# A-SHOJAEI/adverse-weather-semantic-segmentation-robustness-benchmark

Hardware: AMD Instinct MI355X
Metric: images/sec (1024x2048, 5 weather conds, ensemble eval) (higher is better)
Workload: dtype f32 (results float32; attention, gemm_1x1, winograd_3x3, segformer_head on 3xf16 split operands: 22-bit operands, f32 accumulate)

## Files before the change

adverse_weather_semantic_segmentation_robustness_benchmark_amd/_native.py:

```python
from __future__ import annotations

import ctypes as C
from pathlib import Path

import numpy as np
import torch

_PKG = Path(__file__).resolve().parent
LIB_PATH = _PKG / "libawseg_hip.so"

U8, I64 = 0, 1
COMBINE_WEIGHTED, COMBINE_MAXCONF, COMBINE_MEAN = 0, 1, 2
LOSS_CE, LOSS_FOCAL = 0, 1
ACT_NONE, ACT_RELU, ACT_GELU = 0, 1, 2
MAX_CLASSES = 32

c_i, c_i64, c_u64, c_f, c_d, c_p = C.c_int, C.c_int64, C.c_uint64, C.c_float, C.c_double, C.c_void_p

FOG_JOB = np.dtype([("image", "<i4"), ("_pad", "<i4"), ("beta", "<f8"), ("atmos", "<f8"), ("seed", "<u8")], align=True)
NIGHT_JOB = np.dtype([("image", "<i4"), ("_pad", "<i4"), ("brightness", "<f8"), ("intensity", "<f8"), ("seed", "<u8")], align=True)
PRIM_JOB = np.dtype([("image", "<i4"), ("prim_offset", "<i4"), ("prim_count", "<i4"), ("blur_ksize", "<i4"), ("intensity", "<f8")], align=True)
WEATHER_JOB = np.dtype([("kind", "<i4"), ("image", "<i4"), ("a", "<f8"), ("b", "<f8"), ("seed", "<u8"), ("prim_offset", "<i4"), ("prim_count", "<i4")], align=True)
WEATHER_CLEAN, WEATHER_FOG, WEATHER_RAIN, WEATHER_SNOW, WEATHER_NIGHT = 0, 1, 2, 3, 4
assert FOG_JOB.itemsize == 32 and NIGHT_JOB.itemsize == 32 and PRIM_JOB.itemsize == 24 and WEATHER_JOB.itemsize == 40
# ... 12 lines not shown
    "awseg_normalize": (c_i, [c_p, c_i64, c_i, c_i, c_p, c_i, c_p, c_p, c_p, c_p]),
    "awseg_synthetic_depth": (c_i, [c_i, c_i, c_p, c_i, c_p, c_p, c_p, c_p]),
    "awseg_conv3x3_winograd_nhwc": (c_i, [c_p, c_i, c_i, c_i, c_i, c_i, c_i, c_p, c_p, c_p, c_i, c_p, c_p, c_p, c_p]),
    "awseg_gemm_bias_act": (c_i, [c_p, c_p, c_p, c_p, c_i, c_p, c_i64, c_i, c_i, c_p, C.c_size_t, c_p]),
    "awseg_gemm_tune": (c_i, [c_p, c_p, c_p, c_i, c_i, c_p, c_i64, c_i, c_i, c_p, C.c_size_t, c_p]),
    "awseg_gemm_split_weights": (c_i, [c_p, c_i, c_i, c_p, c_p]),
    "awseg_gemm_split_weight_halfs": (c_i64, [c_i, c_i]),
    "awseg_gemm_split_bias_act": (c_i, [c_p, c_p, c_p, c_p, c_i, c_p, c_i64, c_i, c_i, c_p]),
    "awseg_gemm_bf16_weights": (c_i, [c_p, c_i, c_i, c_p, c_p]),
    "awseg_gemm_bf16_weight_halfs": (c_i64, [c_i, c_i]),
    "awseg_gemm_bf16_bias_act": (c_i, [c_p, c_p, c_p, c_p, c_i, c_p, c_i64, c_i, c_i, c_p]),
    "awseg_conv3x3_winograd_bf16_nhwc": (c_i, [c_p, c_i, c_i, c_i, c_i, c_i, c_i, c_p, c_p, c_p, c_i, c_p, c_p, c_p, c_p]),
    "awseg_attention_d32_bf16": (c_i, [c_p, c_p, c_p, c_p, c_i, c_i, c_i, c_i, c_f, c_p]),
    "awseg_attention_d32_split_workspace": (c_i64, [c_i, c_i, c_i]),
    "awseg_attention_d32_split_ws": (c_i, [c_p, c_p, c_p, c_i, c_p, c_i, c_i, c_i, c_i, c_f, c_p, c_p]),
    "awseg_attention_d32_packed_kv": (c_i, [c_p, c_p, c_p, c_i, c_i, c_i, c_i, c_f, c_i, c_p]),
    "awseg_dwconv3x3_upcat_nhwc": (c_i, [c_p, c_i, c_i, c_i, c_p, c_i, c_i64, c_i, c_i, c_p, c_p, c_p]),
    "awseg_winograd_split_weight_halfs": (c_i64, [c_i, c_i]),
    "awseg_conv3x3_winograd_split_nhwc": (c_i, [c_p, c_i, c_i, c_i, c_i, c_i, c_i, c_p, c_p, c_p, c_i, c_p, c_p, c_p, c_p]),
    "awseg_upconv_forms_floats": (c_i64, [c_i, c_i, c_i]),
    "awseg_upconv_forms": (c_i, [c_p, c_i, c_i, c_i, c_i, c_p, c_p, c_p]),
    "awseg_depth_head_fused": (c_i, [c_p, c_i, c_i, c_i, c_i, c_p, c_i, c_p, c_p, c_p, c_p, c_p]),
    "awseg_im2col_nhwc": (c_i, [c_p, c_i64, c_i, c_i, c_i, c_i, c_i, c_i, c_i, c_i, c_i, c_p, c_p]),
    "awseg_attention_d32": (c_i, [c_p, c_p, c_p, c_p, c_i, c_i, c_i, c_i, c_f, c_p]),
    "awseg_attention_d32_split": (c_i, [c_p, c_p, c_p, c_p, c_i, c_i, c_i, c_i, c_f, c_p]),
    "awseg_depth_upsample_combine": (c_i, [c_p, c_p, c_i, c_i, c_i, c_i, c_i, c_p, c_p, c_p, c_p]),
    "awseg_lut3_apply": (c_i, [c_p, c_i, c_i, c_i, c_p, c_i, c_p, c_p, c_p]),
    "awseg_local_contrast": (c_i, [c_p, c_i, c_i, c_i, c_p, c_p]),
    "awseg_depth_estimate_workspace": (C.c_size_t, [c_i]),
    "awseg_depth_estimate": (c_i, [c_p, c_i, c_i, c_i, c_p, c_p, c_p, c_p, c_p]),
# ... 173 lines not shown
```

adverse_weather_semantic_segmentation_robustness_benchmark_amd/csrc/attn.hip:

```cpp
#include "awseg_common.h"

namespace {

typedef float f32x16 __attribute__((ext_vector_type(16)));

constexpr int AT = 256;
#ifndef AWSEG_ATTN_SPLIT_WAVES
#define AWSEG_ATTN_SPLIT_WAVES 2
#endif
constexpr int D = 32;
constexpr int TK = 32;
constexpr int LDK = 36;

__device__ __forceinline__ constexpr int acc_row(int r, int hk) { return (r & 3) + 8 * (r >> 2) + 4 * hk; }

__global__ __launch_bounds__(AT, 2)
void attention_d32_kernel(const float* __restrict__ q, const float* __restrict__ k, const float* __restrict__ v,
                          float* __restrict__ out, int nq, int nkv, int heads, float scale_log2e, int kvp)
{
    __shared__ float sK[2][TK * LDK];
    __shared__ float sV[2][D * LDK];
    const int tid = threadIdx.x, lane = tid & 63, wave = tid >> 6;
    const int hk = lane >> 5, li = lane & 31;
    const int h = blockIdx.y, b = blockIdx.z;
// ... 362 lines not shown
    if (!attn_split_pass<false>(q, k, v, out, nq, nkv, heads, scale_log2e, kvp, sK, sV, sMax, one)) return;
    const int eq = guard_exponent(sMax[0]), ek = guard_exponent(sMax[1]), ev = guard_exponent(sMax[2]);
    auto p2 = [](int e) { return __builtin_bit_cast(float, (unsigned)(127 + e) << 23); };
    const attn_scales sc = {p2(-eq), p2(-ek), p2(-ev), p2(eq), p2(ek), p2(ev)};
    attn_split_pass<true>(q, k, v, out, nq, nkv, heads, scale_log2e, kvp, sK, sV, sMax, sc);
}

constexpr int IMG_TILE_HALFS = (TK + D) * SROW;

__device__ __forceinline__ uint32_t at_lds_addr(const void* p) { return (uint32_t)(uintptr_t)(__attribute__((address_space(3))) const void*)p; }
__device__ __forceinline__ void at_dma16(__amdgpu_buffer_rsrc_t rsrc, uint32_t voff, uint32_t soff, uint32_t lds_base)
{
    asm volatile("s_mov_b32 m0, %3\n\ts_nop 0\n\tbuffer_load_dwordx4 %0, %1, %2 offen lds" : : "v"(voff), "s"(rsrc), "s"(soff), "s"(lds_base) : "m0", "memory");
}

__global__ __launch_bounds__(AT)
void attn_kv_image_kernel(const float* __restrict__ k, const float* __restrict__ v, int kvp, int nkv, int heads,
                          _Float16* __restrict__ img, int* __restrict__ exps)
{
    __shared__ unsigned sM[2];
    const int tid = threadIdx.x, h = blockIdx.x, b = blockIdx.y;
    const float* kb = k + (size_t)b * nkv * kvp + h * D;
    const float* vb = v + (size_t)b * nkv * kvp + h * D;
    const int lkey = tid >> 3, lc = tid & 7;
    const size_t g_off = (size_t)lkey * kvp + 4 * lc;
    const int wk0 = lkey * SROW + 4 * lc;
    const int wv0 = TK * SROW + (4 * lc) * SROW + pv_slot(lkey);
    const int ntiles = nkv / TK;
    if (tid < 2) sM[tid] = 0u;
    __syncthreads();
    float kmax = 0.f, vmax = 0.f;
    for (int t = 0; t < ntiles; ++t) {
        kmax = amax4(kmax, *reinterpret_cast<const float4*>(kb + (size_t)t * TK * kvp + g_off));
        vmax = amax4(vmax, *reinterpret_cast<const float4*>(vb + (size_t)t * TK * kvp + g_off));
    }
    if (kmax >= kSplitLimit) atomicMax(&sM[0], __builtin_bit_cast(unsigned, kmax));
    if (vmax >= kSplitLimit) atomicMax(&sM[1], __builtin_bit_cast(unsigned, vmax));
    __syncthreads();
    const int ek = guard_exponent(sM[0]), ev = guard_exponent(sM[1]);
    auto p2 = [](int e) { return __builtin_bit_cast(float, (unsigned)(127 + e) << 23); };
    const float sk = p2(-ek), sv = p2(-ev);
    if (tid == 0) { exps[((size_t)b * heads + h) * 2] = ek; exps[((size_t)b * heads + h) * 2 + 1] = ev; }
    _Float16* base = img + ((size_t)b * heads + h) * ntiles * IMG_TILE_HALFS;
    for (int t = 0; t < ntiles; ++t) {
        float4 kk4 = *reinterpret_cast<const float4*>(kb + (size_t)t * TK * kvp + g_off);
        float4 vv4 = *reinterpret_cast<const float4*>(vb + (size_t)t * TK * kvp + g_off);
        kk4.x *= sk; kk4.y *= sk; kk4.z *= sk; kk4.w *= sk;
        vv4.x *= sv; vv4.y *= sv; vv4.z *= sv; vv4.w *= sv;
        _Float16* T = base + (size_t)t * IMG_TILE_HALFS;
        u32x2 H, L; unsigned hh, ll;
        split_pair(kk4.x, kk4.y, hh, ll); H[0] = hh; L[0] = ll;
        split_pair(kk4.z, kk4.w, hh, ll); H[1] = hh; L[1] = ll;
        *reinterpret_cast<u32x2*>(&T[wk0]) = H;
        *reinterpret_cast<u32x2*>(&T[wk0 + 32]) = L;
        unsigned vh01, vl01, vh23, vl23;
        split_pair(vv4.x, vv4.y, vh01, vl01);
        split_pair(vv4.z, vv4.w, vh23, vl23);
        unsigned short* sv16 = reinterpret_cast<unsigned short*>(&T[wv0]);
        sv16[0] = (unsigned short)vh01;            sv16[32] = (unsigned short)vl01;
        sv16[SROW] = (unsigned short)(vh01 >> 16); sv16[SROW + 32] = (unsigned short)(vl01 >> 16);
        sv16[2 * SROW] = (unsigned short)vh23;     sv16[2 * SROW + 32] = (unsigned short)vl23;
        sv16[3 * SROW] = (unsigned short)(vh23 >> 16); sv16[3 * SROW + 32] = (unsigned short)(vl23 >> 16);
    }
}

template <bool SCALED, bool QGUARD>
__device__ __forceinline__ bool attn_split_pass_img(const float* __restrict__ q, const _Float16* __restrict__ img_bh, float* __restrict__ out,
                                                    int nq, int nkv, int heads, float scale_log2e, _Float16 (*sKV)[IMG_TILE_HALFS],
                                                    unsigned* sMax, const attn_scales sc)
{
    const int tid = threadIdx.x, lane = tid & 63, wave = tid >> 6;
    const int hk = lane >> 5, li = lane & 31;
    const int h = blockIdx.y, b = blockIdx.z;
    const int C = heads * D;
    const int q0 = blockIdx.x * 128 + wave * 32;
    float qmax = 0.f;
    h8 qh[2], ql[2];
    {
        const int qi = q0 + li;
        const float* qp = q + ((size_t)b * nq + (qi < nq ? qi : nq - 1)) * C + h * D;
        const float qs = SCALED ? scale_log2e * sc.sq : scale_log2e;
#pragma unroll
        for (int s = 0; s < 2; ++s) {
            const float4 a4 = *reinterpret_cast<const float4*>(qp + 16 * s + 8 * hk);
            const float4 b4 = *reinterpret_cast<const float4*>(qp + 16 * s + 8 * hk + 4);
            const float x[8] = { a4.x * qs, a4.y * qs, a4.z * qs, a4.w * qs, b4.x * qs, b4.y * qs, b4.z * qs, b4.w * qs };
            if (QGUARD) {
#pragma unroll
                for (int i = 0; i < 8; ++i) qmax = __builtin_fmaxf(qmax, __builtin_fabsf(x[i]));
            }
            split8(x, qh[s], ql[s]);
        }
    }
// ... 4 lines not shown
    auto dma_tile = [&](int t, int buf) {
        const uint32_t so = (uint32_t)t * (uint32_t)(IMG_TILE_HALFS * 2), lb = lds0 + (uint32_t)buf * (uint32_t)(IMG_TILE_HALFS * 2);
        at_dma16(rsrc, (uint32_t)(lane * 16) + wave_u * 1024u, so, lb + wave_u * 1024u);
        at_dma16(rsrc, (uint32_t)(lane * 16) + (wave_u + 4u) * 1024u, so, lb + (wave_u + 4u) * 1024u);
        if (wave_u == 0) at_dma16(rsrc, (uint32_t)(lane * 16) + 8192u, so, lb + 8192u);
    };
    dma_tile(0, 0);
    asm volatile("s_waitcnt vmcnt(0)" ::: "memory");
    __syncthreads();

    f32x16 om, oc;
#pragma unroll
    for (int r = 0; r < 16; ++r) { om[r] = 0.f; oc[r] = 0.f; }
    float m_run = -1e30f, l_run = 0.f;
    const int a_off = li * SROW + 8 * hk;

    for (int t = 0; t < ntiles; ++t) {
        const int buf = t & 1;
        if (t + 1 < ntiles) dma_tile(t + 1, buf ^ 1);
        const h8* kr = reinterpret_cast<const h8*>(&sKV[buf][a_off]);
        const h8 kh0 = kr[0], kh1 = kr[2], kl0 = kr[4], kl1 = kr[6];
        f32x16 sm, scx;
#pragma unroll
        for (int r = 0; r < 16; ++r) { sm[r] = 0.f; scx[r] = 0.f; }
        sm = __builtin_amdgcn_mfma_f32_32x32x16_f16(kh0, qh[0], sm, 0, 0, 0);
        scx = __builtin_amdgcn_mfma_f32_32x32x16_f16(kh0, ql[0], scx, 0, 0, 0);
        sm = __builtin_amdgcn_mfma_f32_32x32x16_f16(kh1, qh[1], sm, 0, 0, 0);
        scx = __builtin_amdgcn_mfma_f32_32x32x16_f16(kh1, ql[1], scx, 0, 0, 0);
        scx = __builtin_amdgcn_mfma_f32_32x32x16_f16(kl0, qh[0], scx, 0, 0, 0);
        scx = __builtin_amdgcn_mfma_f32_32x32x16_f16(kl1, qh[1], scx, 0, 0, 0);
        const h8* vr = reinterpret_cast<const h8*>(&sKV[buf][TK * SROW + a_off]);
        const h8 vh0 = vr[0], vh1 = vr[2], vl0 = vr[4], vl1 = vr[6];
        float s[16];
#pragma unroll
        for (int r = 0; r < 16; ++r) {
            s[r] = fmaf(scx[r], kLoInv, sm[r]);
            if (SCALED) s[r] = s[r] * sc.bq * sc.bk;
        }
        float mt = fmaxf(fmaxf(s[0], s[1]), fmaxf(s[2], s[3]));
#pragma unroll
        for (int r = 4; r < 16; r += 4) mt = fmaxf(mt, fmaxf(fmaxf(s[r], s[r + 1]), fmaxf(s[r + 2], s[r + 3])));
        mt = fmaxf(mt, __shfl_xor(mt, 32, 64));
        const float m_new = fmaxf(m_run, mt);
        const float alpha = __builtin_amdgcn_exp2f(m_run - m_new);
        const float m_sh = m_new - 15.0f;
        float p[16], ls = 0.f;
// ... 11 lines not shown
        split8_unscaled(p + 8, ph1, pl1);
        om = __builtin_amdgcn_mfma_f32_32x32x16_f16(vh0, ph0, om, 0, 0, 0);
        oc = __builtin_amdgcn_mfma_f32_32x32x16_f16(vl0, ph0, oc, 0, 0, 0);
        om = __builtin_amdgcn_mfma_f32_32x32x16_f16(vh1, ph1, om, 0, 0, 0);
        oc = __builtin_amdgcn_mfma_f32_32x32x16_f16(vl1, ph1, oc, 0, 0, 0);
        om = __builtin_amdgcn_mfma_f32_32x32x16_f16(vh0, pl0, om, 0, 0, 0);
        om = __builtin_amdgcn_mfma_f32_32x32x16_f16(vh1, pl1, om, 0, 0, 0);
        asm volatile("s_waitcnt vmcnt(0)" ::: "memory");
        __syncthreads();
    }

    if (QGUARD) {
        if (qmax >= kSplitLimit) atomicMax(&sMax[0], __builtin_bit_cast(unsigned, qmax));
        __syncthreads();
        if (sMax[0] != 0u) return true;
    }
    const int qi = q0 + li;
    if (qi < nq) {
        const float inv = 1.0f / l_run;
        float* op = out + ((size_t)b * nq + qi) * C + h * D;
#pragma unroll
        for (int g = 0; g < 4; ++g) {
            float4 o4 = make_float4(fmaf(oc[4 * g], kLoInv, om[4 * g]) * inv, fmaf(oc[4 * g + 1], kLoInv, om[4 * g + 1]) * inv,
                                    fmaf(oc[4 * g + 2], kLoInv, om[4 * g + 2]) * inv, fmaf(oc[4 * g + 3], kLoInv, om[4 * g + 3]) * inv);
            if (SCALED) { o4.x *= sc.bv; o4.y *= sc.bv; o4.z *= sc.bv; o4.w *= sc.bv; }
            *reinterpret_cast<float4*>(op + 8 * g + 4 * hk) = o4;
        }
    }
    return false;
}
// ... 8 lines not shown
    if (threadIdx.x == 0) sMax[0] = 0u;
    const _Float16* img_bh = img + ((size_t)b * heads + h) * (size_t)(nkv / TK) * IMG_TILE_HALFS;
    const int ek = exps[((size_t)b * heads + h) * 2], ev = exps[((size_t)b * heads + h) * 2 + 1];
    auto p2 = [](int e) { return __builtin_bit_cast(float, (unsigned)(127 + e) << 23); };
    attn_scales sc = {1.f, p2(-ek), p2(-ev), 1.f, p2(ek), p2(ev)};
    bool redo;
    if ((ek | ev) == 0) redo = attn_split_pass_img<false, true>(q, img_bh, out, nq, nkv, heads, scale_log2e, sKV, sMax, sc);
    else redo = attn_split_pass_img<true, true>(q, img_bh, out, nq, nkv, heads, scale_log2e, sKV, sMax, sc);
    if (!redo) return;
    const int eq = guard_exponent(sMax[0]);
    sc.sq = p2(-eq); sc.bq = p2(eq);
    __syncthreads();
    attn_split_pass_img<true, false>(q, img_bh, out, nq, nkv, heads, scale_log2e, sKV, sMax, sc);
}

__global__ __launch_bounds__(AT, 2)
void attention_d32_bf16_kernel(const float* __restrict__ q, const float* __restrict__ k, const float* __restrict__ v,
                               float* __restrict__ out, int nq, int nkv, int heads, float scale_log2e, int kvp)
{
    __shared__ __attribute__((aligned(16))) _Float16 sK[2][TK * SROW];
    __shared__ __attribute__((aligned(16))) _Float16 sV[2][D * SROW];
    __shared__ unsigned sMax[3];
    const attn_scales one = {1.f, 1.f, 1.f, 1.f, 1.f, 1.f};
    attn_split_pass<false, true>(q, k, v, out, nq, nkv, heads, scale_log2e, kvp, sK, sV, sMax, one);
}

}

namespace {
template <typename K>
// ... 42 lines not shown

AWSEG_API int awseg_attention_d32_split_ws(const float* q, const float* k, const float* v, int kv_pitch, float* out, int batch, int heads,
                                           int n_queries, int n_keys, float scale, void* workspace, awseg_stream_t stream)
{
    if (batch == 0 || n_queries == 0) return 0;
    if (!q || !k || !v || !out || !workspace || batch < 0 || heads < 1 || n_queries < 0 || n_keys < TK) return AWSEG_EINVAL;
    if (n_keys % TK) return AWSEG_ERANGE;
    if (heads > 65535 || batch > 65535) return AWSEG_ERANGE;
    if (((uintptr_t)q & 15) || ((uintptr_t)k & 15) || ((uintptr_t)v & 15) || ((uintptr_t)out & 15) || ((uintptr_t)workspace & 255)) return AWSEG_EALIGN;
    if (kv_pitch == 0) kv_pitch = heads * D;
    if (kv_pitch < heads * D || (kv_pitch & 3)) return AWSEG_EINVAL;
    if ((int64_t)(n_keys / TK) * IMG_TILE_HALFS * 2 > 0x7fffffff) return AWSEG_ERANGE;
    int* exps = reinterpret_cast<int*>(workspace);
    const int64_t tab = ((int64_t)batch * heads * 2 * 4 + 255) / 256 * 256;
    _Float16* img = reinterpret_cast<_Float16*>(reinterpret_cast<char*>(workspace) + tab);
    hipLaunchKernelGGL(attn_kv_image_kernel, dim3((unsigned)heads, (unsigned)batch), dim3(AT), 0, awseg_s(stream), k, v, kv_pitch, n_keys, heads, img, exps);
    AWSEG_LAUNCH_CHECK();
    dim3 grid((unsigned)((n_queries + 127) / 128), (unsigned)heads, (unsigned)batch);
    hipLaunchKernelGGL(attention_d32_split_img_kernel, grid, dim3(AT), 0, awseg_s(stream), q, img, exps, out, n_queries, n_keys, heads,
                       scale * 1.4426950408889634f);
    AWSEG_LAUNCH_CHECK();
    return 0;
}

AWSEG_API int awseg_attention_d32_packed_kv(const float* q, const float* kv, float* out, int batch, int heads, int n_queries,
                                            int n_keys, float scale, int mode, awseg_stream_t stream)
{
    if (!kv) return AWSEG_EINVAL;
    const int c = heads * D;
    switch (mode) {
    case 0: return launch_attention(attention_d32_kernel, q, kv, kv + c, out, batch, heads, n_queries, n_keys, scale, stream, 2 * c);
    case 1: return launch_attention(attention_d32_split_kernel, q, kv, kv + c, out, batch, heads, n_queries, n_keys, scale, stream, 2 * c);
    case 2: return launch_attention(attention_d32_bf16_kernel, q, kv, kv + c, out, batch, heads, n_queries, n_keys, scale, stream, 2 * c);
    default: return AWSEG_EINVAL;
    }
// ... 2 lines not shown
```

adverse_weather_semantic_segmentation_robustness_benchmark_amd/models/fused.py:

```python
from __future__ import annotations

import contextlib
import os
from typing import List

import torch
import torch.nn as nn
import torch.nn.functional as F

from .. import _native as N
from .. import ops

CL = torch.channels_last


def _pair(v):
    return (v, v) if isinstance(v, int) else tuple(v)


def _versions(*tensors):
    return tuple((t.data_ptr(), t._version) for t in tensors if t is not None)


DERIVED = ("wsplit", "wbf16", "wsplit_small", "kvsplit", "proj_pieces", "stemrows")
# ... 339 lines not shown
    if lin.bias is not None and x.is_contiguous() and (ops.gemm_wants_bf16(m, lin.out_features, k) or
                                                       (LINEAR_SPLIT and ops.gemm_wants_split(m, lin.out_features, k))):
        y = ops.gemm_bias_act(x.view(m, k), lin.weight, lin.bias, N.ACT_NONE, w_split=split_weights(lin, lin.weight, m))
        return y.view(*x.shape[:-1], lin.out_features)
    return F.linear(x, lin.weight, lin.bias)


def _linear_residual(x2: torch.Tensor, lin: nn.Linear, tok: torch.Tensor) -> torch.Tensor:
    if lin.bias is None or not tok.is_contiguous():
        return tok + F.linear(x2, lin.weight, lin.bias).view_as(tok)
    t2 = tok.view(-1, tok.shape[-1])
    ops.gemm_bias_act(x2, lin.weight, lin.bias, N.ACT_NONE, residual=t2, out=t2, w_split=split_weights(lin, lin.weight, x2.shape[0]))
    return tok


def _kv_packed(kv: torch.Tensor, a) -> torch.Tensor:
    kp, vp = a.k_proj, a.v_proj
    wkv, bkv = cached(a, "kvpack", [kp.weight, kp.bias, vp.weight, vp.bias],
                      lambda: (torch.cat([kp.weight, vp.weight]).contiguous(), torch.cat([kp.bias, vp.bias]).contiguous()))
    c = kv.shape[-1]
    m = kv.numel() // c
    if ops.gemm_wants_bf16(m, 2 * c, c) or ops.gemm_wants_split(m, 2 * c, c):
        y = ops.gemm_bias_act(kv.view(m, c), wkv, bkv, N.ACT_NONE, w_split=split_weights(a, wkv, m))
    else:
        ws = cached(a, "kvsplit", (wkv,), lambda: ops.gemm_split_weights(wkv))
        y = ops.gemm_bias_act(kv.view(m, c), wkv, bkv, N.ACT_NONE, w_split=ws, split=True)
    return y.view(*kv.shape[:-1], 2 * c)


@torch.no_grad()
# ... 5 lines not shown
    for st in seg.stages:
        pe = st.patch_embeddings
        if _is_patch_gemm(pe.proj) and pe.proj.bias is not None:
            w2 = cached(pe.proj, "patch", [pe.proj.weight], lambda: patch_weights(pe.proj))
            y = conv_gemm_nhwc(nhwc_view(t), pe.proj, w2, pe.proj.bias, N.ACT_NONE)
        else:
            y = _stem_rows(t, pe.proj, pe.proj.weight, pe.proj.bias) if pe.proj.bias is not None else None
            if y is None:
                w = cached(pe.proj, "wcl", [pe.proj.weight], lambda: pe.proj.weight.contiguous(memory_format=CL))
                y = nhwc_view(F.conv2d(t.contiguous(memory_format=CL), w, pe.proj.bias, pe.proj.stride, pe.proj.padding))
        tok = _ln(y, pe.layer_norm)
        B, H, W, C = tok.shape
        for blk in st.blocks:
            a = blk.attention
            hcur = _ln(tok, blk.layernorm_before)
            q = _linear(hcur, a.q_proj)
            if a.sequence_reduction_ratio > 1:
                sr = a.sequence_reduction
                src = sr.sequence_reduction
                if _is_patch_gemm(src) and src.bias is not None:
                    w2 = cached(src, "patch", [src.weight], lambda: patch_weights(src))
                    kv = conv_gemm_nhwc(hcur, src, w2, src.bias, N.ACT_NONE)
                else:
                    wsr = cached(src, "wcl", [src.weight], lambda: src.weight.contiguous(memory_format=CL))
                    kv = nhwc_view(F.conv2d(hcur.permute(0, 3, 1, 2), wsr, src.bias, src.stride))
                kv = _ln(kv, sr.layer_norm)
            else:
                kv = hcur
            nh, d = a.num_attention_heads, a.head_dim
            nkv = kv.shape[1] * kv.shape[2]
            if (d == 32 and nkv % 32 == 0 and ops.KV_PACKED and kv.is_cuda and kv.dtype == torch.float32 and C % 8 == 0
                    and a.k_proj.bias is not None and a.v_proj.bias is not None and kv.is_contiguous()):
                o = ops.attention_d32_packed_kv(q.view(B, H * W, C), _kv_packed(kv, a).view(B, nkv, 2 * C), nh, a.scaling).view(B * H * W, C)
            elif d == 32 and nkv % 32 == 0:
                k, v = _linear(kv, a.k_proj), _linear(kv, a.v_proj)
                o = ops.attention_d32(q.view(B, H * W, C), k.reshape(B, nkv, C), v.reshape(B, nkv, C), nh, a.scaling).view(B * H * W, C)
            else:
                k, v = _linear(kv, a.k_proj), _linear(kv, a.v_proj)
                qq, kk, vv = (t_.view(B, -1, nh, d).transpose(1, 2) for t_ in (q.view(B, H * W, C), k.reshape(B, -1, C), v.reshape(B, -1, C)))
                if ops.PRECISION == "bf16":
                    o = F.scaled_dot_product_attention(qq.bfloat16(), kk.bfloat16(), vv.bfloat16(), scale=a.scaling).float()
                else:
                    o = F.scaled_dot_product_attention(qq, kk, vv, scale=a.scaling)
                o = o.transpose(1, 2).reshape(B * H * W, C)
            tok = _linear_residual(o, a.o_proj, tok)
            m = blk.mlp
            ln2 = blk.layernorm_after
            if (ops.MIXFFN_FUSED and tok.is_cuda and tok.dtype == torch.float32 and C in (32, 64)
                    and getattr(seg.config, "hidden_act", "gelu") == "gelu" and m.fc1.bias is not None and m.fc2.bias is not None
                    and m.dwconv.dwconv.bias is not None and ln2.weight is not None and ln2.bias is not None):
                prep = cached(m, "mixffn", [ln2.weight, ln2.bias, m.fc1.weight, m.fc2.weight],
                              lambda: (ops.mixffn_split_weights(m.fc1.weight), ops.mixffn_split_weights(m.fc2.weight))
                              if ops.mixffn_operands_ok(ln2.weight, ln2.bias, m.fc1.weight, m.fc2.weight) else None)
                fusedtok = None if prep is None else ops.mixffn_fused(
                    tok, ln2.weight, ln2.bias, ln2.eps, m.fc1.weight, m.fc1.bias, dw_taps(m.dwconv.dwconv), m.dwconv.dwconv.bias,
                    m.fc2.weight, m.fc2.bias, w1_split=prep[0], w2_split=prep[1], checked=True)
                if fusedtok is not None:
                    tok = fusedtok
                    continue
            hcur = _linear(_ln(tok, blk.layernorm_after), m.fc1)
# ... 9 lines not shown
```

adverse_weather_semantic_segmentation_robustness_benchmark_amd/ops.py:

```python
from __future__ import annotations

import math
import os

import ctypes as C
from typing import Optional, Sequence

import numpy as np
import torch

from . import _native as N

IMAGENET_MEAN = np.array([0.485, 0.456, 0.406], dtype=np.float32)
IMAGENET_STD = np.array([0.229, 0.224, 0.225], dtype=np.float32)
NIGHT_GAINS = np.array([0.8, 0.85, 1.2], dtype=np.float32)
CONDITIONS = ("clean", "fog", "rain", "snow", "night")


def gaussian_taps(sigma: float = 2.0, truncate: float = 4.0) -> np.ndarray:
    radius = int(truncate * float(sigma) + 0.5)
    x = np.arange(-radius, radius + 1)
    phi = np.exp(-0.5 / (sigma * sigma) * x ** 2)
    return phi / phi.sum()

# ... 1221 lines not shown
    if split is None and PRECISION == "bf16":
        sym = "awseg_attention_d32_bf16"
    else:
        sym = "awseg_attention_d32_split" if (ATTENTION_SPLIT if split is None else split) else "awseg_attention_d32"
    if sym == "awseg_attention_d32_split" and _wants_kv_image(nq, k.shape[1]):
        _attention_split_ws(q, k, v, 0, out, b, heads, nq, k.shape[1], scale)
        return out
    N.call(sym, N.ptr(q), N.ptr(k), N.ptr(v), N.ptr(out), b, heads, nq, k.shape[1], float(scale), N.stream())
    return out


ATTN_KV_IMAGE = os.environ.get("AWSEG_ATTN_KV_IMAGE", "1") != "0"


def _wants_kv_image(nq: int, nkv: int) -> bool:
    return ATTN_KV_IMAGE and nq >= 8 * nkv


def _attention_split_ws(q, k, v, pitch, out, b, heads, nq, nkv, scale):
    nbytes = int(N.lib().awseg_attention_d32_split_workspace(b, heads, nkv))
    ws = N.workspace.get(q.device, nbytes, tag="attn%d" % torch.cuda.current_stream(q.device).cuda_stream)
    N.call("awseg_attention_d32_split_ws", N.ptr(q), N.ptr_strided(k), N.ptr_strided(v), int(pitch), N.ptr(out), b, heads, nq, nkv, float(scale),
           N.ptr(ws), N.stream())


def attention_d32_packed_kv(q: torch.Tensor, kv: torch.Tensor, heads: int, scale: float, split: Optional[bool] = None) -> torch.Tensor:
    q, kv = q.contiguous(), kv.contiguous()
    b, nq, c = q.shape
    assert kv.shape[-1] == 2 * c
    out = torch.empty_like(q)
    mode = 2 if (split is None and PRECISION == "bf16") else (1 if (ATTENTION_SPLIT if split is None else split) else 0)
    if mode == 1 and _wants_kv_image(nq, kv.shape[1]):
        _attention_split_ws(q, kv, kv[..., c:], 2 * c, out, b, heads, nq, kv.shape[1], scale)
        return out
    N.call("awseg_attention_d32_packed_kv", N.ptr(q), N.ptr(kv), N.ptr(out), b, heads, nq, kv.shape[1], float(scale), mode, N.stream())
    return out


# ... 140 lines not shown
```

include/awseg.h:

```cpp
#ifndef AWSEG_H
#define AWSEG_H

#include <stddef.h>
#include <stdint.h>

#ifdef __cplusplus
extern "C" {
#endif

typedef void* awseg_stream_t;

#define AWSEG_EINVAL   (-1)
#define AWSEG_ERANGE   (-2)
#define AWSEG_EALIGN   (-3)

#define AWSEG_U8   0
#define AWSEG_I64  1

#define AWSEG_COMBINE_WEIGHTED  0
#define AWSEG_COMBINE_MAXCONF   1
#define AWSEG_COMBINE_MEAN      2

#define AWSEG_LOSS_CE     0
#define AWSEG_LOSS_FOCAL  1
// ... 218 lines not shown
                                        const float* bias, const float* residual, int act, float* out, int n,
                                        awseg_stream_t stream);

int64_t awseg_gemm_bf16_weight_halfs(int n, int k);
int awseg_gemm_bf16_weights(const float* w, int n, int k, uint16_t* w_bf16, awseg_stream_t stream);
int awseg_gemm_bf16_bias_act(const float* x, const uint16_t* w_bf16, const float* bias, const float* residual, int act,
                             float* out, int64_t m, int n, int k, awseg_stream_t stream);
int awseg_conv3x3_winograd_bf16_nhwc(const float* x, int batch, int height, int width, int cin, int cout, int dilation,
                                     const uint16_t* u_bf16, const float* shift, const float* residual, int act,
                                     const float* w2, const float* b2, float* out, awseg_stream_t stream);
int awseg_attention_d32_bf16(const float* q, const float* k, const float* v, float* out, int batch, int heads,
                             int n_queries, int n_keys, float scale, awseg_stream_t stream);
int64_t awseg_attention_d32_split_workspace(int batch, int heads, int n_keys);
int awseg_attention_d32_split_ws(const float* q, const float* k, const float* v, int kv_pitch, float* out, int batch, int heads,
                                 int n_queries, int n_keys, float scale, void* workspace, awseg_stream_t stream);

int awseg_attention_d32_packed_kv(const float* q, const float* kv, float* out, int batch, int heads, int n_queries,
                                  int n_keys, float scale, int mode, awseg_stream_t stream);

int awseg_upconv3x3_linear(const float* g9, int64_t batch, int cmid, int h, int w, int height, int width,
                           const float* bias, float* out, int channels_last, awseg_stream_t stream);
int awseg_upconv3x3_adjoint(const float* dz, int64_t batch, int cmid, int h, int w, int height, int width,
                            float* dg9, awseg_stream_t stream);

int awseg_im2col_nhwc(const float* x, int64_t batch, int height, int width, int channels, int kernel_h, int kernel_w,
                      int stride, int pad, int dilation, int k_padded, float* cols, awseg_stream_t stream);

int awseg_attention_d32(const float* q, const float* k, const float* v, float* out, int batch, int heads,
                        int n_queries, int n_keys, float scale, awseg_stream_t stream);

// ... 159 lines not shown
```

Baseline: 235.6.

## Fuse Q and output projections into the single-head d32 attention kernel

Adds a fused attention kernel for single-head, 32-channel stages. It computes the Q projection from the layernorm output in registers via split-f16 MFMA, runs the KV-image attention, then applies the output projection plus residual directly into the token buffer. This removes two separate GEMM launches and the round trips of q and o through global memory. The KV image builder is also spread across several tile-blocks per head and stages tiles in LDS for coalesced stores, and the KV-image threshold is lowered to nq >= 4*nkv. The cost is more register pressure and extra in-kernel block reductions for the dynamic input scaling.

```diff
diff --git a/adverse_weather_semantic_segmentation_robustness_benchmark_amd/_native.py b/adverse_weather_semantic_segmentation_robustness_benchmark_amd/_native.py
--- a/adverse_weather_semantic_segmentation_robustness_benchmark_amd/_native.py
+++ b/adverse_weather_semantic_segmentation_robustness_benchmark_amd/_native.py
@@ -50,6 +50,7 @@
     "awseg_attention_d32_bf16": (c_i, [c_p, c_p, c_p, c_p, c_i, c_i, c_i, c_i, c_f, c_p]),
     "awseg_attention_d32_split_workspace": (c_i64, [c_i, c_i, c_i]),
     "awseg_attention_d32_split_ws": (c_i, [c_p, c_p, c_p, c_i, c_p, c_i, c_i, c_i, c_i, c_f, c_p, c_p]),
+    "awseg_attention_d32_proj_ws": (c_i, [c_p, c_p, c_p, c_p, c_p, c_p, c_p, c_i, c_p, c_i, c_i, c_i, c_i, c_i, c_f, c_p, c_p]),
     "awseg_attention_d32_packed_kv": (c_i, [c_p, c_p, c_p, c_i, c_i, c_i, c_i, c_f, c_i, c_p]),
     "awseg_dwconv3x3_upcat_nhwc": (c_i, [c_p, c_i, c_i, c_i, c_p, c_i, c_i64, c_i, c_i, c_p, c_p, c_p]),
     "awseg_winograd_split_weight_halfs": (c_i64, [c_i, c_i]),
diff --git a/adverse_weather_semantic_segmentation_robustness_benchmark_amd/csrc/attn.hip b/adverse_weather_semantic_segmentation_robustness_benchmark_amd/csrc/attn.hip
--- a/adverse_weather_semantic_segmentation_robustness_benchmark_amd/csrc/attn.hip
+++ b/adverse_weather_semantic_segmentation_robustness_benchmark_amd/csrc/attn.hip
@@ -400,12 +400,15 @@
     asm volatile("s_mov_b32 m0, %3\n\ts_nop 0\n\tbuffer_load_dwordx4 %0, %1, %2 offen lds" : : "v"(voff), "s"(rsrc), "s"(soff), "s"(lds_base) : "m0", "memory");
 }
 
+constexpr int IMG_TILES_PER_BLOCK = 4;
+
 __global__ __launch_bounds__(AT)
 void attn_kv_image_kernel(const float* __restrict__ k, const float* __restrict__ v, int kvp, int nkv, int heads,
                           _Float16* __restrict__ img, int* __restrict__ exps)
 {
+    __shared__ __attribute__((aligned(16))) _Float16 sT[2][IMG_TILE_HALFS];
     __shared__ unsigned sM[2];
-    const int tid = threadIdx.x, h = blockIdx.x, b = blockIdx.y;
+    const int tid = threadIdx.x, h = blockIdx.y, b = blockIdx.z;
     const float* kb = k + (size_t)b * nkv * kvp + h * D;
     const float* vb = v + (size_t)b * nkv * kvp + h * D;
     const int lkey = tid >> 3, lc = tid & 7;
@@ -413,9 +416,19 @@
     const int wk0 = lkey * SROW + 4 * lc;
     const int wv0 = TK * SROW + (4 * lc) * SROW + pv_slot(lkey);
     const int ntiles = nkv / TK;
+    const int t0 = blockIdx.x * IMG_TILES_PER_BLOCK;
+    const int nt = ntiles - t0 < IMG_TILES_PER_BLOCK ? ntiles - t0 : IMG_TILES_PER_BLOCK;
     if (tid < 2) sM[tid] = 0u;
     __syncthreads();
+    float4 kk[IMG_TILES_PER_BLOCK], vv[IMG_TILES_PER_BLOCK];
+#pragma unroll
+    for (int i = 0; i < IMG_TILES_PER_BLOCK; ++i) {
+        const int t = t0 + (i < nt ? i : 0);
+        kk[i] = *reinterpret_cast<const float4*>(kb + (size_t)t * TK * kvp + g_off);
+        vv[i] = *reinterpret_cast<const float4*>(vb + (size_t)t * TK * kvp + g_off);
+    }
     float kmax = 0.f, vmax = 0.f;
+#pragma unroll 8
     for (int t = 0; t < ntiles; ++t) {
         kmax = amax4(kmax, *reinterpret_cast<const float4*>(kb + (size_t)t * TK * kvp + g_off));
         vmax = amax4(vmax, *reinterpret_cast<const float4*>(vb + (size_t)t * TK * kvp + g_off));
@@ -426,14 +439,16 @@
     const int ek = guard_exponent(sM[0]), ev = guard_exponent(sM[1]);
     auto p2 = [](int e) { return __builtin_bit_cast(float, (unsigned)(127 + e) << 23); };
     const float sk = p2(-ek), sv = p2(-ev);
-    if (tid == 0) { exps[((size_t)b * heads + h) * 2] = ek; exps[((size_t)b * heads + h) * 2 + 1] = ev; }
-    _Float16* base = img + ((size_t)b * heads + h) * ntiles * IMG_TILE_HALFS;
-    for (int t = 0; t < ntiles; ++t) {
-        float4 kk4 = *reinterpret_cast<const float4*>(kb + (size_t)t * TK * kvp + g_off);
-        float4 vv4 = *reinterpret_cast<const float4*>(vb + (size_t)t * TK * kvp + g_off);
+    if (tid == 0 && blockIdx.x == 0) { exps[((size_t)b * heads + h) * 2] = ek; exps[((size_t)b * heads + h) * 2 + 1] = ev; }
+    _Float16* base = img + (((size_t)b * heads + h) * ntiles + t0) * IMG_TILE_HALFS;
+    const int c0 = (tid >> 3) * SROW + (tid & 7) * 8, c1 = c0 + (AT >> 3) * SROW;
+#pragma unroll
+    for (int i = 0; i < IMG_TILES_PER_BLOCK; ++i) {
+        if (i >= nt) break;
+        float4 kk4 = kk[i], vv4 = vv[i];
         kk4.x *= sk; kk4.y *= sk; kk4.z *= sk; kk4.w *= sk;
         vv4.x *= sv; vv4.y *= sv; vv4.z *= sv; vv4.w *= sv;
-        _Float16* T = base + (size_t)t * IMG_TILE_HALFS;
+        _Float16* T = sT[i & 1];
         u32x2 H, L; unsigned hh, ll;
         split_pair(kk4.x, kk4.y, hh, ll); H[0] = hh; L[0] = ll;
         split_pair(kk4.z, kk4.w, hh, ll); H[1] = hh; L[1] = ll;
@@ -447,13 +462,92 @@
         sv16[SROW] = (unsigned short)(vh01 >> 16); sv16[SROW + 32] = (unsigned short)(vl01 >> 16);
         sv16[2 * SROW] = (unsigned short)vh23;     sv16[2 * SROW + 32] = (unsigned short)vl23;
         sv16[3 * SROW] = (unsigned short)(vh23 >> 16); sv16[3 * SROW + 32] = (unsigned short)(vl23 >> 16);
-    }
-}
-
-template <bool SCALED, bool QGUARD>
+        __syncthreads();
+        _Float16* G = base + (size_t)i * IMG_TILE_HALFS;
+        *reinterpret_cast<u32x4*>(&G[c0]) = *reinterpret_cast<const u32x4*>(&T[c0]);
+        *reinterpret_cast<u32x4*>(&G[c1]) = *reinterpret_cast<const u32x4*>(&T[c1]);
+    }
+}
+
+struct attn_proj_args {
+    const float* x;
+    const uint16_t* wq3; const unsigned* wq_trailer; const float* bq;
+    const uint16_t* wo3; const unsigned* wo_trailer; const float* bo;
+    float* tok;
+};
+constexpr float kProjScale0 = 16.0f;
+constexpr int kProjExp0 = -4;
+constexpr float kProjBig = 2048.0f, kProjSmall = 0.0078125f;
+
+__device__ __forceinline__ float at_pow2(int e) { return __builtin_bit_cast(float, (unsigned)(127 + e) << 23); }
+__device__ __forceinline__ void proj_split2(float a, float b, float s, unsigned& hi, unsigned& lo)
+{
+    asm("v_fma_mixlo_f16 %0, %2, %4, 0\n\t"
+        "v_fma_mixhi_f16 %0, %3, %4, 0\n\t"
+        "v_fma_mixlo_f16 %1, %2, %4, -%0 op_sel_hi:[0,0,1]\n\t"
+        "v_fma_mixhi_f16 %1, %3, %4, -%0 op_sel:[0,0,1] op_sel_hi:[0,0,1]\n\t"
+        "s_nop 1"
+        : "=&v"(hi), "=&v"(lo) : "v"(a), "v"(b), "v"(s));
+}
+template <bool RES>
+__device__ __forceinline__ void proj_rows32(const float (&x)[16], const uint16_t* __restrict__ w3, const unsigned* __restrict__ trailer,
+                                            const float* __restrict__ bias, const float (&res)[16], unsigned* sM, int lane, float (&y)[16])
+{
+    const int hk = lane >> 5, li = lane & 31;
+    float amax = 0.f;
+#pragma unroll
+    for (int i = 0; i < 16; ++i) amax = __builtin_fmaxf(amax, __builtin_fabsf(x[i]));
+#pragma unroll
+    for (int o = 32; o > 0; o >>= 1) amax = __builtin_fmaxf(amax, __shfl_xor(amax, o, 64));
+    if (lane == 0) atomicMax(sM, __builtin_bit_cast(unsigned, amax));
+    __syncthreads();
+    const unsigned mx = *sM;
+    int xe = kProjExp0; float sx = kProjScale0;
+    constexpr unsigned kBig = __builtin_bit_cast(unsigned, kProjBig), kSmall = __builtin_bit_cast(unsigned, kProjSmall);
+    if (mx >= kBig || (mx >= 0x00800000u && mx < kSmall)) {
+        const int ex = (int)(mx >> 23) & 0xff;
+        if (ex != 0xff) {
+            xe = ex - 127 - 13;
+            xe = xe < -127 ? -127 : xe;
+            sx = at_pow2(-xe);
+        }
+    }
+    const uint16_t* wrow = w3 + pv_slot(li) * 64 + 8 * hk;
+    f32x16 acc;
+#pragma unroll
+    for (int r = 0; r < 16; ++r) acc[r] = 0.f;
+#pragma unroll
+    for (int s = 0; s < 2; ++s) {
+        const h8 wh = *reinterpret_cast<const h8*>(wrow + 16 * s), wl = *reinterpret_cast<const h8*>(wrow + 32 + 16 * s);
+        u32x4 H, L;
+#pragma unroll
+        for (int i = 0; i < 4; ++i) { unsigned h, l; proj_split2(x[8 * s + 2 * i], x[8 * s + 2 * i + 1], sx, h, l); H[i] = h; L[i] = l; }
+        const h8 xh = __builtin_bit_cast(h8, H), xl = __builtin_bit_cast(h8, L);
+        acc = __builtin_amdgcn_mfma_f32_32x32x16_f16(wh, xh, acc, 0, 0, 0);
+        acc = __builtin_amdgcn_mfma_f32_32x32x16_f16(wl, xh, acc, 0, 0, 0);
+        acc = __builtin_amdgcn_mfma_f32_32x32x16_f16(wh, xl, acc, 0, 0, 0);
+    }
+    const int oe = (int)trailer[1] + xe;
+    const int oe1 = oe / 2, oe2 = oe - oe1;
+    const float os1 = at_pow2(oe1 < -126 ? -126 : (oe1 > 127 ? 127 : oe1)), os2 = at_pow2(oe2 < -126 ? -126 : (oe2 > 127 ? 127 : oe2));
+#pragma unroll
+    for (int s = 0; s < 2; ++s) {
+        const float4 b0 = *reinterpret_cast<const float4*>(bias + 16 * s + 8 * hk), b1 = *reinterpret_cast<const float4*>(bias + 16 * s + 8 * hk + 4);
+        const float bb[8] = { b0.x, b0.y, b0.z, b0.w, b1.x, b1.y, b1.z, b1.w };
+#pragma unroll
+        for (int j = 0; j < 8; ++j) {
+            float vv = acc[8 * s + j] * os1 * os2;
+            vv = vv + bb[j];
+            if (RES) vv = vv + res[8 * s + j];
+            y[8 * s + j] = __builtin_fmaxf(vv, -__builtin_inff());
+        }
+    }
+}
+
+template <bool SCALED, bool QGUARD, bool PROJ = false>
 __device__ __forceinline__ bool attn_split_pass_img(const float* __restrict__ q, const _Float16* __restrict__ img_bh, float* __restrict__ out,
                                                     int nq, int nkv, int heads, float scale_log2e, _Float16 (*sKV)[IMG_TILE_HALFS],
-                                                    unsigned* sMax, const attn_scales sc)
+                                                    unsigned* sMax, const attn_scales sc, const attn_proj_args& pa = attn_proj_args{})
 {
     const int tid = threadIdx.x, lane = tid & 63, wave = tid >> 6;
     const int hk = lane >> 5, li = lane & 31;
@@ -462,7 +556,30 @@
     const int q0 = blockIdx.x * 128 + wave * 32;
     float qmax = 0.f;
     h8 qh[2], ql[2];
-    {
+    if constexpr (PROJ) {
+        const float* xp = pa.x + ((size_t)b * nq + q0 + li) * D;
+        float xv[16], qv[16];
+#pragma unroll
+        for (int s = 0; s < 2; ++s) {
+            const float4 a4 = *reinterpret_cast<const float4*>(xp + 16 * s + 8 * hk);
+            const float4 b4 = *reinterpret_cast<const float4*>(xp + 16 * s + 8 * hk + 4);
+            xv[8 * s] = a4.x; xv[8 * s + 1] = a4.y; xv[8 * s + 2] = a4.z; xv[8 * s + 3] = a4.w;
+            xv[8 * s + 4] = b4.x; xv[8 * s + 5] = b4.y; xv[8 * s + 6] = b4.z; xv[8 * s + 7] = b4.w;
+        }
+        proj_rows32<false>(xv, pa.wq3, pa.wq_trailer, pa.bq, xv, &sMax[1], lane, qv);
+        const float qs = SCALED ? scale_log2e * sc.sq : scale_log2e;
+#pragma unroll
+        for (int s = 0; s < 2; ++s) {
+            float x[8];
+#pragma unroll
+            for (int i = 0; i < 8; ++i) x[i] = qv[8 * s + i] * qs;
+            if (QGUARD) {
+#pragma unroll
+                for (int i = 0; i < 8; ++i) qmax = __builtin_fmaxf(qmax, __builtin_fabsf(x[i]));
+            }
+            split8(x, qh[s], ql[s]);
+        }
+    } else {
         const int qi = q0 + li;
         const float* qp = q + ((size_t)b * nq + (qi < nq ? qi : nq - 1)) * C + h * D;
         const float qs = SCALED ? scale_log2e * sc.sq : scale_log2e;
@@ -497,6 +614,7 @@
     for (int r = 0; r < 16; ++r) { om[r] = 0.f; oc[r] = 0.f; }
     float m_run = -1e30f, l_run = 0.f;
     const int a_off = li * SROW + 8 * hk;
+    const int v_off = PROJ ? pv_slot(li) * SROW + 8 * hk : a_off;
 
     for (int t = 0; t < ntiles; ++t) {
         const int buf = t & 1;
@@ -512,7 +630,7 @@
         scx = __builtin_amdgcn_mfma_f32_32x32x16_f16(kh1, ql[1], scx, 0, 0, 0);
         scx = __builtin_amdgcn_mfma_f32_32x32x16_f16(kl0, qh[0], scx, 0, 0, 0);
         scx = __builtin_amdgcn_mfma_f32_32x32x16_f16(kl1, qh[1], scx, 0, 0, 0);
-        const h8* vr = reinterpret_cast<const h8*>(&sKV[buf][TK * SROW + a_off]);
+        const h8* vr = reinterpret_cast<const h8*>(&sKV[buf][TK * SROW + v_off]);
         const h8 vh0 = vr[0], vh1 = vr[2], vl0 = vr[4], vl1 = vr[6];
         float s[16];
 #pragma unroll
@@ -554,6 +672,26 @@
         if (qmax >= kSplitLimit) atomicMax(&sMax[0], __builtin_bit_cast(unsigned, qmax));
         __syncthreads();
         if (sMax[0] != 0u) return true;
+    }
+    if constexpr (PROJ) {
+        const float inv = 1.0f / l_run;
+        float ov[16], rv[16], yv[16];
+#pragma unroll
+        for (int r = 0; r < 16; ++r) {
+            ov[r] = fmaf(oc[r], kLoInv, om[r]) * inv;
+            if (SCALED) ov[r] *= sc.bv;
+        }
+        float* tp = pa.tok + ((size_t)b * nq + q0 + li) * D + 8 * hk;
+#pragma unroll
+        for (int g = 0; g < 4; ++g) {
+            const float4 t4 = *reinterpret_cast<const float4*>(tp + 16 * (g >> 1) + 4 * (g & 1));
+            rv[4 * g] = t4.x; rv[4 * g + 1] = t4.y; rv[4 * g + 2] = t4.z; rv[4 * g + 3] = t4.w;
+        }
+        proj_rows32<true>(ov, pa.wo3, pa.wo_trailer, pa.bo, rv, &sMax[2], lane, yv);
+#pragma unroll
+        for (int g = 0; g < 4; ++g)
+            *reinterpret_cast<float4*>(tp + 16 * (g >> 1) + 4 * (g & 1)) = make_float4(yv[4 * g], yv[4 * g + 1], yv[4 * g + 2], yv[4 * g + 3]);
+        return false;
     }
     const int qi = q0 + li;
     if (qi < nq) {
@@ -592,6 +730,29 @@
     attn_split_pass_img<true, false>(q, img_bh, out, nq, nkv, heads, scale_log2e, sKV, sMax, sc);
 }
 
+__global__ __launch_bounds__(AT, AWSEG_ATTN_SPLIT_WAVES)
+void attention_d32_proj_img_kernel(const attn_proj_args pa, const _Float16* __restrict__ img, const int* __restrict__ exps,
+                                   int nq, int nkv, float scale_log2e)
+{
+    __shared__ __attribute__((aligned(16))) _Float16 sKV[2][IMG_TILE_HALFS];
+    __shared__ unsigned sMax[3];
+    const int b = blockIdx.z;
+    if (threadIdx.x < 3) sMax[threadIdx.x] = 0u;
+    __syncthreads();
+    const _Float16* img_bh = img + (size_t)b * (size_t)(nkv / TK) * IMG_TILE_HALFS;
+    const int ek = exps[(size_t)b * 2], ev = exps[(size_t)b * 2 + 1];
+    auto p2 = [](int e) { return __builtin_bit_cast(float, (unsigned)(127 + e) << 23); };
+    attn_scales sc = {1.f, p2(-ek), p2(-ev), 1.f, p2(ek), p2(ev)};
+    bool redo;
+    if ((ek | ev) == 0) redo = attn_split_pass_img<false, true, true>(nullptr, img_bh, nullptr, nq, nkv, 1, scale_log2e, sKV, sMax, sc, pa);
+    else redo = attn_split_pass_img<true, true, true>(nullptr, img_bh, nullptr, nq, nkv, 1, scale_log2e, sKV, sMax, sc, pa);
+    if (!redo) return;
+    const int eq = guard_exponent(sMax[0]);
+    sc.sq = p2(-eq); sc.bq = p2(eq);
+    __syncthreads();
+    attn_split_pass_img<true, false, true>(nullptr, img_bh, nullptr, nq, nkv, 1, scale_log2e, sKV, sMax, sc, pa);
+}
+
 __global__ __launch_bounds__(AT, 2)
 void attention_d32_bf16_kernel(const float* __restrict__ q, const float* __restrict__ k, const float* __restrict__ v,
                                float* __restrict__ out, int nq, int nkv, int heads, float scale_log2e, int kvp)
@@ -664,11 +825,39 @@
     int* exps = reinterpret_cast<int*>(workspace);
     const int64_t tab = ((int64_t)batch * heads * 2 * 4 + 255) / 256 * 256;
     _Float16* img = reinterpret_cast<_Float16*>(reinterpret_cast<char*>(workspace) + tab);
-    hipLaunchKernelGGL(attn_kv_image_kernel, dim3((unsigned)heads, (unsigned)batch), dim3(AT), 0, awseg_s(stream), k, v, kv_pitch, n_keys, heads, img, exps);
+    hipLaunchKernelGGL(attn_kv_image_kernel, dim3((unsigned)((n_keys / TK + IMG_TILES_PER_BLOCK - 1) / IMG_TILES_PER_BLOCK), (unsigned)heads, (unsigned)batch), dim3(AT), 0, awseg_s(stream), k, v, kv_pitch, n_keys, heads, img, exps);
     AWSEG_LAUNCH_CHECK();
     dim3 grid((unsigned)((n_queries + 127) / 128), (unsigned)heads, (unsigned)batch);
     hipLaunchKernelGGL(attention_d32_split_img_kernel, grid, dim3(AT), 0, awseg_s(stream), q, img, exps, out, n_queries, n_keys, heads,
                        scale * 1.4426950408889634f);
+    AWSEG_LAUNCH_CHECK();
+    return 0;
+}
+
+AWSEG_API int awseg_attention_d32_proj_ws(const float* x, const uint16_t* wq_split, const float* bq, const uint16_t* wo_split, const float* bo,
+                                          const float* k, const float* v, int kv_pitch, float* tok, int batch, int heads, int channels,
+                                          int n_queries, int n_keys, float scale, void* workspace, awseg_stream_t stream)
+{
+    if (batch == 0 || n_queries == 0) return 0;
+    if (!x || !wq_split || !bq || !wo_split || !bo || !k || !v || !tok || !workspace || batch < 0 || heads < 1 || n_queries < 0 || n_keys < TK) return AWSEG_EINVAL;
+    if (heads != 1 || channels != D || n_queries % 128 || n_keys % TK || batch > 65535) return AWSEG_ERANGE;
+    if (((uintptr_t)x & 15) || ((uintptr_t)wq_split & 15) || ((uintptr_t)wo_split & 15) || ((uintptr_t)bq & 15) || ((uintptr_t)bo & 15) ||
+        ((uintptr_t)k & 15) || ((uintptr_t)v & 15) || ((uintptr_t)tok & 15) || ((uintptr_t)workspace & 255)) return AWSEG_EALIGN;
+    if (kv_pitch == 0) kv_pitch = D;
+    if (kv_pitch < D || (kv_pitch & 3)) return AWSEG_EINVAL;
+    if ((int64_t)(n_keys / TK) * IMG_TILE_HALFS * 2 > 0x7fffffff) return AWSEG_ERANGE;
+    int* exps = reinterpret_cast<int*>(workspace);
+    const int64_t tab = ((int64_t)batch * 2 * 4 + 255) / 256 * 256;
+    _Float16* img = reinterpret_cast<_Float16*>(reinterpret_cast<char*>(workspace) + tab);
+    hipLaunchKernelGGL(attn_kv_image_kernel, dim3((unsigned)((n_keys / TK + IMG_TILES_PER_BLOCK - 1) / IMG_TILES_PER_BLOCK), 1u, (unsigned)batch), dim3(AT), 0,
+                       awseg_s(stream), k, v, kv_pitch, n_keys, 1, img, exps);
+    AWSEG_LAUNCH_CHECK();
+    attn_proj_args pa;
+    pa.x = x; pa.tok = tok; pa.bq = bq; pa.bo = bo;
+    pa.wq_trailer = reinterpret_cast<const unsigned*>(wq_split + 2 * D * D); pa.wq3 = wq_split + 2 * D * D + 8;
+    pa.wo_trailer = reinterpret_cast<const unsigned*>(wo_split + 2 * D * D); pa.wo3 = wo_split + 2 * D * D + 8;
+    hipLaunchKernelGGL(attention_d32_proj_img_kernel, dim3((unsigned)(n_queries / 128), 1u, (unsigned)batch), dim3(AT), 0, awseg_s(stream), pa, img, exps,
+                       n_queries, n_keys, scale * 1.4426950408889634f);
     AWSEG_LAUNCH_CHECK();
     return 0;
 }
diff --git a/adverse_weather_semantic_segmentation_robustness_benchmark_amd/models/fused.py b/adverse_weather_semantic_segmentation_robustness_benchmark_amd/models/fused.py
--- a/adverse_weather_semantic_segmentation_robustness_benchmark_amd/models/fused.py
+++ b/adverse_weather_semantic_segmentation_robustness_benchmark_amd/models/fused.py
@@ -377,6 +377,17 @@
     return tok
 
 
+def _attn_proj_routed(a, hcur: torch.Tensor, tok: torch.Tensor) -> bool:
+    B, H, W, C = tok.shape
+    m = B * H * W
+    sr = a.sequence_reduction_ratio
+    nkv = (H // sr) * (W // sr) if sr > 1 else H * W
+    return (a.head_dim == 32 and nkv % 32 == 0 and ops.KV_PACKED and tok.is_cuda and tok.dtype == torch.float32 and tok.is_contiguous()
+            and hcur.is_contiguous() and a.q_proj.bias is not None and a.o_proj.bias is not None and a.k_proj.bias is not None
+            and a.v_proj.bias is not None and LINEAR_SPLIT and ops.gemm_wants_split(m, C, C) and not ops.gemm_wants_bf16(m, C, C)
+            and ops.attn_proj_routes(m, a.num_attention_heads, C, H * W, ops._cus(tok.device)))
+
+
 def _kv_packed(kv: torch.Tensor, a) -> torch.Tensor:
     kp, vp = a.k_proj, a.v_proj
     wkv, bkv = cached(a, "kvpack", [kp.weight, kp.bias, vp.weight, vp.bias],
@@ -412,7 +423,8 @@
         for blk in st.blocks:
             a = blk.attention
             hcur = _ln(tok, blk.layernorm_before)
-            q = _linear(hcur, a.q_proj)
+            proj = _attn_proj_routed(a, hcur, tok)
+            q = None if proj else _linear(hcur, a.q_proj)
             if a.sequence_reduction_ratio > 1:
                 sr = a.sequence_reduction
                 src = sr.sequence_reduction
@@ -429,11 +441,22 @@
             nkv = kv.shape[1] * kv.shape[2]
             if (d == 32 and nkv % 32 == 0 and ops.KV_PACKED and kv.is_cuda and kv.dtype == torch.float32 and C % 8 == 0
                     and a.k_proj.bias is not None and a.v_proj.bias is not None and kv.is_contiguous()):
-                o = ops.attention_d32_packed_kv(q.view(B, H * W, C), _kv_packed(kv, a).view(B, nkv, 2 * C), nh, a.scaling).view(B * H * W, C)
+                kvp = _kv_packed(kv, a).view(B, nkv, 2 * C)
+                if proj:
+                    ops.attention_d32_proj(hcur.view(B, H * W, C), a.q_proj.weight, a.q_proj.bias, a.o_proj.weight, a.o_proj.bias, kvp,
+                                           tok.view(B, H * W, C), nh, a.scaling, wq_split=split_weights(a.q_proj, a.q_proj.weight, B * H * W),
+                                           wo_split=split_weights(a.o_proj, a.o_proj.weight, B * H * W))
+                    o = None
+                else:
+                    if q is None:
+                        q = _linear(hcur, a.q_proj)
+                    o = ops.attention_d32_packed_kv(q.view(B, H * W, C), kvp, nh, a.scaling).view(B * H * W, C)
             elif d == 32 and nkv % 32 == 0:
+                q = _linear(hcur, a.q_proj) if q is None else q
                 k, v = _linear(kv, a.k_proj), _linear(kv, a.v_proj)
                 o = ops.attention_d32(q.view(B, H * W, C), k.reshape(B, nkv, C), v.reshape(B, nkv, C), nh, a.scaling).view(B * H * W, C)
             else:
+                q = _linear(hcur, a.q_proj) if q is None else q
                 k, v = _linear(kv, a.k_proj), _linear(kv, a.v_proj)
                 qq, kk, vv = (t_.view(B, -1, nh, d).transpose(1, 2) for t_ in (q.view(B, H * W, C), k.reshape(B, -1, C), v.reshape(B, -1, C)))
                 if ops.PRECISION == "bf16":
@@ -441,7 +464,8 @@
                 else:
                     o = F.scaled_dot_product_attention(qq, kk, vv, scale=a.scaling)
                 o = o.transpose(1, 2).reshape(B * H * W, C)
-            tok = _linear_residual(o, a.o_proj, tok)
+            if o is not None:
+                tok = _linear_residual(o, a.o_proj, tok)
             m = blk.mlp
             ln2 = blk.layernorm_after
             if (ops.MIXFFN_FUSED and tok.is_cuda and tok.dtype == torch.float32 and C in (32, 64)
diff --git a/adverse_weather_semantic_segmentation_robustness_benchmark_amd/ops.py b/adverse_weather_semantic_segmentation_robustness_benchmark_amd/ops.py
--- a/adverse_weather_semantic_segmentation_robustness_benchmark_amd/ops.py
+++ b/adverse_weather_semantic_segmentation_robustness_benchmark_amd/ops.py
@@ -1259,7 +1259,7 @@
 
 
 def _wants_kv_image(nq: int, nkv: int) -> bool:
-    return ATTN_KV_IMAGE and nq >= 8 * nkv
+    return ATTN_KV_IMAGE and nq >= 4 * nkv
 
 
 def _attention_split_ws(q, k, v, pitch, out, b, heads, nq, nkv, scale):
@@ -1267,6 +1267,59 @@
     ws = N.workspace.get(q.device, nbytes, tag="attn%d" % torch.cuda.current_stream(q.device).cuda_stream)
     N.call("awseg_attention_d32_split_ws", N.ptr(q), N.ptr_strided(k), N.ptr_strided(v), int(pitch), N.ptr(out), b, heads, nq, nkv, float(scale),
            N.ptr(ws), N.stream())
+
+
+ATTN_PROJ = os.environ.get("AWSEG_ATTN_PROJ", "1") != "0"
+
+
+def gemm_split_rows128(m: int, n: int, k: int, cus: int) -> bool:
+    bn = 256 if n % 256 == 0 else (128 if n % 128 == 0 else (64 if n >= 8 else 0))
+    if bn == 0 or k % 8 or k < 32 or m < 1:
+        return False
+    t256, t128 = (m + 255) // 256, (m + 127) // 128
+    if not (t256 * ((n + bn - 1) // bn) >= cus // 2 or t128 * ((n + 127) // 128) >= cus // 2):
+        return False
+    bn_half = 128 if bn >= 128 else 64
+    few = t256 * ((n + bn - 1) // bn) < cus
+    return few or ((k <= 128 or (bn <= 128 and k <= 512)) and t128 * ((n + bn_half - 1) // bn_half) >= 4 * cus)
+
+
+def attn_proj_routes(m: int, heads: int, c: int, nq: int, cus: int) -> bool:
+    if not (ATTN_PROJ and ATTENTION_SPLIT and ATTN_KV_IMAGE and GEMM_SPLIT and PRECISION == "f32"):
+        return False
+    if heads != 1 or c != 32 or nq < 128 or nq % 128 or m % nq:
+        return False
+    return gemm_split_rows128(m, 32, 32, cus)
+
+
+def _cus(device) -> int:
+    return torch.cuda.get_device_properties(device).multi_processor_count
+
+
+def attention_d32_proj(x: torch.Tensor, wq: torch.Tensor, bq: torch.Tensor, wo: torch.Tensor, bo: torch.Tensor, kv: torch.Tensor,
+                       tok: torch.Tensor, heads: int, scale: float, wq_split: Optional[torch.Tensor] = None,
+                       wo_split: Optional[torch.Tensor] = None) -> torch.Tensor:
+    b, nq, c = x.shape
+    nkv = kv.shape[1]
+    x, kv = x.contiguous(), kv.contiguous()
+    assert tok.is_contiguous() and tok.shape == x.shape and kv.shape[-1] == 2 * c and c == heads * 32
+    wq_split = gemm_split_weights(wq) if wq_split is None else wq_split
+    wo_split = gemm_split_weights(wo) if wo_split is None else wo_split
+    if not (_split_weights_intact(wq_split, c, c) and _split_weights_intact(wo_split, c, c)):
+        raise N.AwsegError("w_split lost its 16-byte trailer (weight exponent): pass the tensor gemm_split_weights returned, not a copy")
+    bq, bo = bq.contiguous(), bo.contiguous()
+    if ATTN_PROJ and not ((bq.data_ptr() | bo.data_ptr() | x.data_ptr() | tok.data_ptr() | kv.data_ptr()) & 15):
+        nbytes = int(N.lib().awseg_attention_d32_split_workspace(b, heads, nkv))
+        ws = N.workspace.get(x.device, nbytes, tag="attn%d" % torch.cuda.current_stream(x.device).cuda_stream)
+        rc = N.try_call("awseg_attention_d32_proj_ws", N.ptr(x), N.ptr(wq_split), N.ptr(bq), N.ptr(wo_split), N.ptr(bo), N.ptr(kv),
+                        N.ptr_strided(kv[..., c:]), 2 * c, N.ptr(tok), b, heads, c, nq, nkv, float(scale), N.ptr(ws), N.stream())
+        if rc == 0:
+            return tok
+    q = gemm_split_bias_act(x.view(b * nq, c), wq_split, bq, 0)
+    o = attention_d32_packed_kv(q.view(b, nq, c), kv, heads, scale, split=True)
+    t2 = tok.view(b * nq, c)
+    gemm_split_bias_act(o.view(b * nq, c), wo_split, bo, 0, residual=t2, out=t2)
+    return tok
 
 
 def attention_d32_packed_kv(q: torch.Tensor, kv: torch.Tensor, heads: int, scale: float, split: Optional[bool] = None) -> torch.Tensor:
diff --git a/include/awseg.h b/include/awseg.h
--- a/include/awseg.h
+++ b/include/awseg.h
@@ -256,6 +256,10 @@
 int64_t awseg_attention_d32_split_workspace(int batch, int heads, int n_keys);
 int awseg_attention_d32_split_ws(const float* q, const float* k, const float* v, int kv_pitch, float* out, int batch, int heads,
                                  int n_queries, int n_keys, float scale, void* workspace, awseg_stream_t stream);
+
+int awseg_attention_d32_proj_ws(const float* x, const uint16_t* wq_split, const float* bq, const uint16_t* wo_split, const float* bo,
+                                const float* k, const float* v, int kv_pitch, float* tok, int batch, int heads, int channels,
+                                int n_queries, int n_keys, float scale, void* workspace, awseg_stream_t stream);
 
 int awseg_attention_d32_packed_kv(const float* q, const float* kv, float* out, int batch, int heads, int n_queries,
                                   int n_keys, float scale, int mode, awseg_stream_t stream);
```

Result: faster. 238.3 (median of 6 runs) (+1.1%).
